# tukaani-project/xz

Measured on AMD Instinct MI355X. Metric: compress MB/s + ratio vs xz -T0 -6, 4 GiB input, 1/2/4/8 MI355X, higher is better.
Workload: dtype u8

## Files before the change

### include/xz_amd.h

```cpp
#ifndef XZ_AMD_H
#define XZ_AMD_H

#include <stddef.h>
#include <stdint.h>

#ifdef __cplusplus
extern "C" {
#endif

typedef struct xzamd_ctx xzamd_ctx;

#define XZAMD_OK              0
#define XZAMD_STREAM_END      1
#define XZAMD_UNSUPPORTED_CHECK 3
#define XZAMD_MEM_ERROR       5
#define XZAMD_OPTIONS_ERROR   8
#define XZAMD_DATA_ERROR      9
#define XZAMD_BUF_ERROR      10
#define XZAMD_PROG_ERROR     11
#define XZAMD_DEVICE_ERROR  100

#define XZAMD_CHECK_NONE   0
#define XZAMD_CHECK_CRC32  1
#define XZAMD_CHECK_CRC64  4
// ... 59 lines not shown
void xzamd_release_parked(void);
uint64_t xzamd_mt_block_size(const xzamd_lzma_options *opt);
uint64_t xzamd_block_buffer_bound(uint64_t uncompressed_size);
uint64_t xzamd_stream_buffer_bound(uint64_t in_size, uint64_t block_size);

int xzamd_ctx_create(xzamd_ctx **ctx, int device);
void xzamd_ctx_destroy(xzamd_ctx *ctx);
int xzamd_ctx_set_batch_bytes(xzamd_ctx *ctx, uint64_t bytes);
const char *xzamd_last_error(const xzamd_ctx *ctx);
int xzamd_ctx_device(const xzamd_ctx *ctx);

typedef struct {
	uint64_t in_bytes, out_bytes;
	uint64_t blocks, spans, batches;
	uint64_t blocks_stored;
	float ms_chains;
	float ms_encode;
	float ms_crc;
	float ms_assemble;
	float ms_total;
	uint32_t encode_launches;
	float ms_find;
	uint32_t span_size;
	float ms_find_overlapped;
	uint32_t span_cost_used;
	float ms_plan;
	uint32_t wave_slots;
	uint64_t enc_spans;
	float ms_seed;
	float ms_parse;
	float ms_code;
	float ms_iter1;
	float ms_verify;
} xzamd_stats;
void xzamd_get_stats(const xzamd_ctx *ctx, xzamd_stats *out);

#define XZAMD_F_BLOCKS_ONLY 1u
#define XZAMD_F_SEGMENTS 2u

#define XZAMD_F_KEEP_RESUME 4u
#define XZAMD_F_VERIFY 8u
#define XZAMD_F_REPAIR 16u
#define XZAMD_F_SINGLE 32u
#define XZAMD_F_AUTO_DELTA 64u

typedef struct {
	uint64_t unpadded_size;
	uint64_t uncompressed_size;
	uint64_t out_offset;
	uint64_t total_size;
} xzamd_block_info;

int xzamd_stream_encode_device(xzamd_ctx *ctx,
		const void *d_in, uint64_t in_size, uint64_t block_size,
		const xzamd_lzma_options *opt, int check, uint32_t flags,
		void *d_out, uint64_t out_cap, uint64_t *out_size,
		xzamd_block_info *binfo, uint64_t binfo_cap, uint64_t *nblocks,
		void *stream);

int xzamd_auto_delta_device(xzamd_ctx *ctx, const void *d_in, uint64_t in_size, uint64_t block_size, uint32_t *dist_out,
		uint64_t cap, uint64_t *nblocks, void *stream);

int xzamd_stream_decode_device(xzamd_ctx *ctx, const void *d_xz, uint64_t xz_size, void *d_out, uint64_t out_cap,
		uint64_t *out_size, const void *d_expected, uint64_t expected_size, uint64_t *mismatches, uint64_t *nblocks,
		void *stream);

// ... 142 lines not shown
```

### xz_amd/__init__.py

```python
import ctypes as C
import os

_HERE = os.path.dirname(os.path.abspath(__file__))
LIB_PATH = os.environ.get("XZ_AMD_LIB") or os.path.join(_HERE, "libxz_amd.so")

CHECK_NONE, CHECK_CRC32, CHECK_CRC64, CHECK_SHA256 = 0, 1, 4, 10
MF_HC3, MF_HC4, MF_BT4 = 0x03, 0x04, 0x14
PRESET_EXTREME = 0x80000000
SPAN_WHOLE_BLOCK = 0xFFFFFFFF
SPAN_DEFAULT = 0
SPAN_AUTO = 1
F_BLOCKS_ONLY = 1
F_SEGMENTS = 2
F_KEEP_RESUME = 4
F_VERIFY = 8
F_REPAIR = 16
F_SINGLE = 32
F_AUTO_DELTA = 64
AUTO_DELTA_DISTANCES = (0, 1, 2, 3, 4, 6, 8, 12, 16, 24, 32)
DEBUG_DELTA_HIST, DEBUG_DELTA_DIST = 19, 20
VSTEPS = ("none", "grammar", "decode", "check", "compare")
NO_BLOCK = 0xFFFFFFFFFFFFFFFF
BCJ_X86 = 4
BCJ_ARM64 = 0x0A
BCJ_RISCV = 0x0B
BCJ_POWERPC, BCJ_IA64, BCJ_ARM, BCJ_ARMTHUMB, BCJ_SPARC = 5, 6, 7, 8, 9


def filter_delta(dist):
    return 3 | ((dist - 1) << 8)



class LzmaOptions(C.Structure):
    _fields_ = [(n, C.c_uint32) for n in (
        "dict_size", "lc", "lp", "pb", "mode", "nice_len", "mf", "depth",
        "gpu_mf", "gpu_nice_len", "gpu_depth", "span_size", "gpu_sa_window", "gpu_parser", "bcj",
        "gpu_sa_depth", "span_cost", "span_bits", "enc_span_bits", "bcj2", "bcj3", "part_iters")]


class Stats(C.Structure):
    _fields_ = [("in_bytes", C.c_uint64), ("out_bytes", C.c_uint64), ("blocks", C.c_uint64),
                ("spans", C.c_uint64), ("batches", C.c_uint64), ("blocks_stored", C.c_uint64),
                ("ms_chains", C.c_float), ("ms_encode", C.c_float), ("ms_crc", C.c_float),
                ("ms_assemble", C.c_float), ("ms_total", C.c_float), ("encode_launches", C.c_uint32),
                ("ms_find", C.c_float), ("span_size", C.c_uint32), ("ms_find_overlapped", C.c_float),
                ("span_cost_used", C.c_uint32), ("ms_plan", C.c_float), ("wave_slots", C.c_uint32),
                ("enc_spans", C.c_uint64), ("ms_seed", C.c_float), ("ms_parse", C.c_float), ("ms_code", C.c_float), ("ms_iter1", C.c_float),
                ("ms_verify", C.c_float)]


class VerifyReport(C.Structure):
    _fields_ = [("units", C.c_uint64), ("blocks", C.c_uint64), ("records_used", C.c_uint64), ("first_bad_block", C.c_uint64),
                ("mismatching_words", C.c_uint64), ("table_used", C.c_uint32), ("first_bad_step", C.c_uint32),
                ("ms_verify", C.c_float), ("reserved_", C.c_uint32)]


class RepairReport(C.Structure):
    _fields_ = [("blocks", C.c_uint64), ("blocks_bad", C.c_uint64), ("blocks_reencoded", C.c_uint64),
                ("blocks_stored", C.c_uint64), ("size_before", C.c_uint64), ("size_after", C.c_uint64),
                ("passes", C.c_uint32), ("ms_repair", C.c_float), ("ms_verify_passes", C.c_float),
                ("ms_reencode", C.c_float), ("ms_splice", C.c_float), ("reserved_", C.c_uint32)]


class ForwardReport(C.Structure):
    _fields_ = [(n, C.c_uint64) for n in ("streams", "blocks", "blocks_delivered", "consumed", "stop_offset")] + \
               [(n, C.c_uint32) for n in ("stop", "code", "step", "reserved_")]


FWD_CONCATENATED = 1
FWD_END, FWD_TRUNCATED, FWD_DEFECT, FWD_OUT_FULL = 1, 2, 3, 4


class BlockInfo(C.Structure):
    _fields_ = [("unpadded_size", C.c_uint64), ("uncompressed_size", C.c_uint64),
                ("out_offset", C.c_uint64), ("total_size", C.c_uint64)]


class XzStream(C.Structure):
    _fields_ = [(n, C.c_uint64) for n in ("offset", "size", "padding", "first_block", "block_count",
                                          "uncompressed_offset", "uncompressed_size")] + \
               [("check", C.c_uint32), ("reserved_", C.c_uint32)]
# ... 527 lines not shown
```

### xz_amd/csrc/xzamd_host.c

```c
#include "../../include/xz_amd.h"
#include "kernels_api.h"
#include "xzamd_internal.h"
#include "delta_rule.h"

#include <stdio.h>
#include <pthread.h>
#include <stdlib.h>
#include <string.h>

#define DEFAULT_BATCH ((1ull << 31) - (1ull << 20))
#define CRC_STRIP 4096u

typedef struct {
	void *p;
	uint64_t cap;
} dbuf;

enum { EV_START, EV_CHAINS, EV_FIND, EV_PLAN0, EV_PLAN1, EV_SEED, EV_ITER1, EV_PARSE, EV_FRONT, EV_BACK0, EV_CODE, EV_CRC, EV_ASM, EV_COUNT };

typedef struct {
	int active;
	uint64_t b0, nb, in_off, n64;
	uint32_t n;
	uint32_t nspans, nenc;
	uint32_t nout, opb;
	uint32_t nch;
	uint64_t sort_bytes;
	int par;
	int sha_early;
	const uint8_t *enc_in;
	uint64_t max_segs, max_lits;
} batch_run;

typedef struct {
	int no_overlap;
	int back_beside_build;
	int timing;
	uint32_t tok_limit, log_cap;
} call_knobs;

typedef struct {
	const xzamd_lzma_options *opt;
	const uint8_t *d_in;
	uint8_t *d_out;
	uint64_t in_size, block_size, out_cap, bound, binfo_cap, total_blocks;
	uint64_t max_blocks;
	uint32_t hb, hmask, hbits;
	uint32_t span;
	uint32_t spb, esb, cpb;
	uint32_t cbytes, hs_fixed;
	uint32_t hs_delta;
	int auto_delta;
	int segments;
	xzamd_mode m;
	call_knobs k;
	int check, whole, filtered, pipelined, defer, seeds_early;
	int resume, verify;
	int repair;
	uint32_t rec_done;
	uint8_t dbyte;
	void *st, *stb;
	uint64_t *rec_unp, *rec_unc;
	xzamd_block_info *binfo;
	uint64_t opos;
} job_env;

struct xzamd_ctx {
	int device;
	void *own_stream;
	void *st2;
	void *st3;
	void *ev_seed[2][3];
	void *ev_sha;
	uint64_t batch_bytes;
	uint32_t wave_slots;
	uint32_t cus;
	uint32_t span_waves;
	uint64_t alloc_limit;
	char err[256];
	char err_msg_buf[200];
	dbuf keys_a, keys_b, vals_a, vals_b, rank, sorted_pos, prev2, prev3, prev4, prev8, prev16, prev24, prev32, key64_a, key64_b, sa, sa_rank, sort_tmp;
	dbuf scratch, span_bytes, strip_crc, block_crc, segs, lits, trace, errw, errw2, litp, mlen, mdist, bcj[2], bcjt;
	dbuf est, totals, span_tab[2], span_cnt[2], mtop, order;
	dbuf pinfo[2], snap_sr, part_tab;
	dbuf cb_bnd[2], cb_log[2], cb_hdr[2], cb_start[2], cb_carry[2];
	dbuf sym_len[2], sym_dist[2], prior, enc_tab[2], enc_cnt[2];
	dbuf tok, chunks, h_chunks;
	dbuf dhist, ddist[2];
	dbuf resume_sr;
	dbuf resume_tab;
	struct { int valid; uint32_t stride, nrec; uint64_t nblocks, block_size, in_size; } resume;
	xzamd_verify_report report;
	xzamd_repair_report repair;
	dbuf h_span_bytes, h_block_crc, h_segs, h_lits, h_span_tab, h_span_cnt[2], h_enc_tab[2], h_enc_cnt[2], h_err[2], h_ddist[2];
	void *evp[2][EV_COUNT];
	void *ev_total[2];
	uint32_t trace_cap;
	int trace_on;
	int last_par;
	struct { int active; job_env J; batch_run B; } pend;
	int pend_has_result, pend_rc;
	uint64_t pend_out_size;
	uint64_t par_seq;
	pthread_mutex_t prog_mu;
// ... 28 lines not shown
		b->p = NULL;
		b->cap = 0;
	}
	bytes = (bytes + 255) & ~255ull;
	if (c->alloc_limit && bytes > c->alloc_limit)
		return fail(c, XZAMD_MEM_ERROR, "allocation above XZAMD_TEST_ALLOC_LIMIT_MIB", 0);
	int e = host ? xzk_host_alloc(&b->p, bytes) : xzk_malloc(&b->p, bytes);
	if (e)
		return fail(c, XZAMD_MEM_ERROR, host ? "hipHostMalloc" : "hipMalloc", e);
	b->cap = bytes;
	return 0;
}

int xzamd_ctx_create(xzamd_ctx **out, int device)
{
	*out = NULL;
	int ndev = 0;
	if (xzk_device_count(&ndev) || ndev <= 0)
		return XZAMD_DEVICE_ERROR;
	xzamd_ctx *c = (xzamd_ctx *)calloc(1, sizeof(*c));
	if (!c)
		return XZAMD_MEM_ERROR;
	if (device < 0) {
		if (xzk_get_device(&device)) { free(c); return XZAMD_DEVICE_ERROR; }
	}
	if (device >= ndev || xzk_set_device(device)) { free(c); return XZAMD_DEVICE_ERROR; }
	c->device = device;
	if (pthread_mutex_init(&c->prog_mu, NULL)) { free(c); return XZAMD_MEM_ERROR; }
	c->prog_mu_ok = 1;
	if (xzk_stream_create(&c->own_stream)) { c->own_stream = NULL; xzamd_ctx_destroy(c); return XZAMD_DEVICE_ERROR; }
	if ((getenv("XZAMD_ST2_LOW") ? xzk_stream_create_low(&c->st2) : xzk_stream_create(&c->st2))) { c->st2 = NULL; xzamd_ctx_destroy(c); return XZAMD_DEVICE_ERROR; }
	if (xzk_event_create(&c->ev_sha)) { c->ev_sha = NULL; xzamd_ctx_destroy(c); return XZAMD_DEVICE_ERROR; }
	if (xzk_stream_create(&c->st3)) { c->st3 = NULL; xzamd_ctx_destroy(c); return XZAMD_DEVICE_ERROR; }
	for (int i = 0; i < 6; ++i)
		if (xzk_event_create(&c->ev_seed[i / 3][i % 3])) { c->ev_seed[i / 3][i % 3] = NULL; xzamd_ctx_destroy(c); return XZAMD_DEVICE_ERROR; }
	for (int i = 0; i < 2 * EV_COUNT; ++i)
		if (xzk_event_create(&c->evp[i / EV_COUNT][i % EV_COUNT])) { c->evp[i / EV_COUNT][i % EV_COUNT] = NULL; xzamd_ctx_destroy(c); return XZAMD_DEVICE_ERROR; }
	for (int i = 0; i < 2; ++i)
		if (xzk_event_create(&c->ev_total[i])) { c->ev_total[i] = NULL; xzamd_ctx_destroy(c); return XZAMD_DEVICE_ERROR; }
	{
		const char *lim = getenv("XZAMD_TEST_ALLOC_LIMIT_MIB");
		c->alloc_limit = (lim && *lim && atoll(lim) > 0) ? (uint64_t)atoll(lim) << 20 : 0;
	}
	c->batch_bytes = DEFAULT_BATCH;
	{
		int cus = 0;
		if (xzk_cu_count(device, &cus) || cus <= 0) cus = 256;
		int occ = 0;
		if (xzk_span_occupancy(1, 64, &occ) || occ <= 0 || occ > 32) occ = 16;
		c->cus = (uint32_t)cus;
		c->wave_slots = (uint32_t)cus * (uint32_t)occ;
		const char *pw = getenv("XZAMD_SPAN_WAVES_PER_CU");
		c->span_waves = (pw && atoi(pw) > 0) ? (uint32_t)cus * (uint32_t)atoi(pw) : 0;
	}
	const char *env = getenv("XZAMD_BATCH_MIB");
	if (env && atoll(env) > 0)
		xzamd_ctx_set_batch_bytes(c, (uint64_t)atoll(env) << 20);
	*out = c;
	return XZAMD_OK;
}

#define CTX_NBUF_MAX 96
static void ctx_device_bufs(xzamd_ctx *c, dbuf **d, size_t *nd)
{
	dbuf *all[] = { &c->keys_a, &c->keys_b, &c->vals_a, &c->vals_b, &c->rank, &c->sorted_pos,
		&c->prev2, &c->prev3, &c->prev4, &c->prev8, &c->prev16, &c->prev24, &c->prev32, &c->key64_a, &c->key64_b, &c->sa, &c->sa_rank, &c->sort_tmp,
// ... 6 lines not shown
		&c->cb_carry[0], &c->cb_carry[1], &c->resume_sr, &c->ddist[0], &c->ddist[1] };
	_Static_assert(sizeof(all) / sizeof(all[0]) <= CTX_NBUF_MAX, "ctx_device_bufs: raise CTX_NBUF_MAX");
	*nd = sizeof(all) / sizeof(all[0]);
	memcpy(d, all, sizeof(all));
}
#define CTX_NBIG 36

void xzamd_ctx_destroy(xzamd_ctx *c)
{
	if (!c)
		return;
	xzk_set_device(c->device);
	if (c->pend.active) {
		if (c->st2) xzk_sync(c->st2);
		c->pend.active = 0;
	}
	dbuf *d[CTX_NBUF_MAX];
	size_t nd = 0;
	ctx_device_bufs(c, d, &nd);
	for (size_t i = 0; i < nd; ++i)
		if (d[i]->p) xzk_free(d[i]->p);
	if (c->resume_tab.p) xzk_free(c->resume_tab.p);
	dbuf *h[] = { &c->h_span_bytes, &c->h_block_crc, &c->h_segs, &c->h_lits, &c->h_span_tab, &c->h_span_cnt[0], &c->h_span_cnt[1],
		&c->h_enc_tab[0], &c->h_enc_tab[1], &c->h_enc_cnt[0], &c->h_enc_cnt[1], &c->h_err[0], &c->h_err[1], &c->h_chunks, &c->h_ddist[0], &c->h_ddist[1] };
	for (size_t i = 0; i < sizeof(h) / sizeof(h[0]); ++i)
		if (h[i]->p) xzk_host_free(h[i]->p);
	for (int i = 0; i < 2 * EV_COUNT; ++i)
		if (c->evp[i / EV_COUNT][i % EV_COUNT]) xzk_event_destroy(c->evp[i / EV_COUNT][i % EV_COUNT]);
	for (int i = 0; i < 2; ++i)
		if (c->ev_total[i]) xzk_event_destroy(c->ev_total[i]);
	if (c->ev_sha) xzk_event_destroy(c->ev_sha);
	for (int i = 0; i < 6; ++i)
		if (c->ev_seed[i / 3][i % 3]) xzk_event_destroy(c->ev_seed[i / 3][i % 3]);
	if (c->st3) xzk_stream_destroy(c->st3);
	if (c->st2) xzk_stream_destroy(c->st2);
	if (c->own_stream) xzk_stream_destroy(c->own_stream);
	if (c->prog_mu_ok) pthread_mutex_destroy(&c->prog_mu);
	free(c);
}

uint64_t xzamd_ctx_progress_in_(xzamd_ctx *c)
{
	if (!c || !c->prog_mu_ok)
		return 0;
	pthread_mutex_lock(&c->prog_mu);
	uint64_t v = c->prog_done;
	if (c->prog_cur) {
		void **ev = c->evp[c->prog_par];
		uint32_t pct = 0;
		if (xzk_event_query(ev[EV_CHAINS]) == 0) {
			pct = 25;
			if (xzk_event_query(ev[EV_FIND]) == 0) {
				pct = 40;
				if (xzk_event_query(ev[EV_PARSE]) == 0)
					pct = xzk_event_query(ev[EV_CODE]) == 0 ? 100 : 90;
			}
		}
		v += c->prog_cur / 100 * pct;
	}
	pthread_mutex_unlock(&c->prog_mu);
	return v;
}

void xzamd_ctx_progress_reset_(xzamd_ctx *c)
{
	if (!c || !c->prog_mu_ok)
// ... 140 lines not shown
	uint8_t *lits; uint64_t lits_len, lits_cap;
	xzamd_copy_seg *segs; uint64_t nsegs, segs_cap;
} plan;

static uint64_t plan_lit(plan *p, const uint8_t *bytes, uint64_t n, uint64_t dst)
{
	memcpy(p->lits + p->lits_len, bytes, n);
	xzamd_copy_seg *s = &p->segs[p->nsegs++];
	s->src = p->lits_len; s->dst = dst; s->len = n; s->kind = 1; s->pad_ = 0;
	p->lits_len += n;
	return dst + n;
}

static uint64_t plan_seg(plan *p, uint32_t kind, uint64_t src, uint64_t n, uint64_t dst)
{
	if (n == 0)
		return dst;
	xzamd_copy_seg *s = &p->segs[p->nsegs++];
	s->src = src; s->dst = dst; s->len = n; s->kind = kind; s->pad_ = 0;
	return dst + n;
}

static uint32_t knob_below(const char *s, uint32_t limit)
{
	const unsigned long v = s ? strtoul(s, NULL, 10) : 0;
	return v >= 1 && v < limit ? (uint32_t)v : 0;
}

static void knobs_read(call_knobs *k)
{
	k->no_overlap = getenv("XZAMD_NO_OVERLAP") != NULL;
	k->back_beside_build = getenv("XZAMD_BACK_BESIDE_BUILD") != NULL;
	k->timing = getenv("XZAMD_TIMING") != NULL;
	k->tok_limit = knob_below(getenv("XZAMD_TEST_TOK_PER_BYTE"), XZAMD_TOK_PER_BYTE);
	k->log_cap = knob_below(getenv("XZAMD_TEST_LOG_CAP"), XZAMD_LOG_CAP);
}

static int call_setup(xzamd_ctx *c, job_env *J, const uint8_t *d_in, uint64_t in_size, uint64_t block_size,
		const xzamd_lzma_options *opt, int check, uint32_t flags, uint8_t *d_out, uint64_t out_cap,
		xzamd_block_info *binfo, uint64_t binfo_cap, void *stream, int may_defer)
{
	if (c->pend_has_result)
		return fail(c, XZAMD_PROG_ERROR, "result of the previous deferred call not collected", 0);
	c->err[0] = 0;
	const uint32_t cbytes = xzamd_check_bytes_(check);
	if (flags & XZAMD_F_SEGMENTS)
		flags |= XZAMD_F_BLOCKS_ONLY;
	if ((unsigned)check > 15)
		return fail(c, XZAMD_PROG_ERROR, "check id out of range", 0);
	const int chains = (flags & XZAMD_F_CHAINS_) != 0;
	if (flags & XZAMD_F_AUTO_DELTA) {
		if (!xzk_delta_stats || !xzk_delta_choose || !xzk_delta_blocks)
			return fail(c, XZAMD_OPTIONS_ERROR, "auto delta: this build has no kernels for it", 0);
		if (opt->bcj != 0)
			return fail(c, XZAMD_OPTIONS_ERROR, "auto delta: the chain already has a filter in front of LZMA2", 0);
		if (flags & XZAMD_F_SEGMENTS)
			return fail(c, XZAMD_OPTIONS_ERROR, "auto delta: Blocks only -- the segments of one Block share its chain", 0);
		if (flags & XZAMD_F_REPAIR)
			return fail(c, XZAMD_OPTIONS_ERROR, "auto delta: not with XZAMD_F_REPAIR (the repair plans Block Headers from one chain)", 0);
	}
	if (chains && (!(flags & XZAMD_F_SEGMENTS) || !xzamd_chains_encoded_))
		return fail(c, XZAMD_OPTIONS_ERROR, "chains: this build has no unit for bare chunk chains", 0);
	if ((flags & XZAMD_F_REPAIR) && (flags & XZAMD_F_SEGMENTS) && !chains)
		return fail(c, XZAMD_OPTIONS_ERROR, "repair: Blocks only, not the chunk chains of XZAMD_F_SEGMENTS", 0);
	if ((flags & (XZAMD_F_KEEP_RESUME | XZAMD_F_VERIFY)) && (flags & XZAMD_F_BLOCKS_ONLY) && !(flags & XZAMD_F_REPAIR) && !chains)
		return fail(c, XZAMD_OPTIONS_ERROR, "keep_resume / verify need a whole Stream: not with XZAMD_F_BLOCKS_ONLY or XZAMD_F_SEGMENTS", 0);
// ... 49 lines not shown
	{
		double per_byte = xzamd_work_bytes_per_byte_(opt);
		if (flags & XZAMD_F_AUTO_DELTA) per_byte += xzamd_auto_delta_bytes_per_byte_(block_size);
		if ((flags & (XZAMD_F_KEEP_RESUME | XZAMD_F_VERIFY)) && J->m.two)
			per_byte += (double)(XZAMD_RESUME_BYTES(J->m.model_slots) + 32u) * (double)(block_size / XZAMD_ENC_MIN_LEN + 1) / (double)block_size;
		uint64_t free_b = 0, total_b = 0, held = 0;
		if (xzk_mem_info(&free_b, &total_b) == 0 && total_b != 0) {
			dbuf *d[CTX_NBUF_MAX];
			size_t nd = 0;
			ctx_device_bufs(c, d, &nd);
			for (size_t i = 0; i < nd; ++i) held += d[i]->cap;
			const double budget = 0.80 * (double)(free_b + held);
			uint64_t fit = (uint64_t)(budget / per_byte) / block_size;
			if (fit == 0) fit = 1;
			if (fit < max_blocks) max_blocks = fit;
		}
	}
	if (total_blocks > max_blocks) {
		const uint64_t nbatch = (total_blocks + max_blocks - 1) / max_blocks;
		max_blocks = (total_blocks + nbatch - 1) / nbatch;
	}
	const int adaptive = J->m.adaptive, two = J->m.two;
	J->spb = adaptive ? (uint32_t)(block_size / XZAMD_SPAN_MIN_LEN + 2) : (uint32_t)((block_size + J->span - 1) / J->span);
	J->esb = two ? (uint32_t)(block_size / XZAMD_ENC_MIN_LEN + 1) : 0;
	J->cpb = (uint32_t)((block_size + XZAMD_EST_CHUNK - 1) / XZAMD_EST_CHUNK);
	J->filtered = opt->bcj != 0;
	J->auto_delta = (flags & XZAMD_F_AUTO_DELTA) != 0;
	const int overlap_ok = two && !J->k.no_overlap;
	J->defer = may_defer && overlap_ok && (flags & XZAMD_F_BLOCKS_ONLY) && total_blocks > 0 && !(flags & (XZAMD_F_REPAIR | XZAMD_F_VERIFY));
	if (c->pend.active && !(overlap_ok && c->pend.J.st == st))
		(void)pend_complete(c);
	J->pipelined = overlap_ok && (total_blocks > max_blocks || J->defer || c->pend.active);
	J->seeds_early = overlap_ok && block_size >= XZAMD_SEED_LEN + 1024;

	J->opt = opt; J->d_in = d_in; J->d_out = d_out; J->in_size = in_size; J->block_size = block_size; J->out_cap = out_cap;
	J->total_blocks = total_blocks; J->max_blocks = max_blocks;
	J->bound = xzamd_block_buffer_bound(block_size);
	J->binfo = binfo; J->binfo_cap = binfo_cap;
	J->cbytes = cbytes; J->hs_fixed = xzamd_block_header_size_(J->bound, block_size, opt);
	if (J->auto_delta) {
		xzamd_lzma_options view = *opt;
		view.bcj = XZAMD_FILTER_DELTA(1);
		J->hs_delta = xzamd_block_header_size_(J->bound, block_size, &view);
	}
	J->check = check;
	J->dbyte = xzamd_dict_size_byte_(opt->dict_size);
	J->st = st; J->stb = J->pipelined ? c->st2 : st;
	J->whole = !(flags & XZAMD_F_BLOCKS_ONLY);
	J->segments = (flags & XZAMD_F_SEGMENTS) != 0;
	J->resume = (flags & (XZAMD_F_KEEP_RESUME | XZAMD_F_VERIFY)) && two;
	J->verify = (flags & XZAMD_F_VERIFY) != 0;
	J->repair = (flags & XZAMD_F_REPAIR) != 0;
	c->resume.valid = 0;
	if (c->resume_tab.p && !J->resume && !c->pend.active) {
		xzk_free(c->resume_tab.p);
		c->resume_tab.p = NULL; c->resume_tab.cap = 0;
	}
	if (J->resume) {
		const uint64_t cap = total_blocks * J->esb;
		if (cap >= 0xFFFFFFFFull)
			return fail(c, XZAMD_OPTIONS_ERROR, "too many encode spans for a resume table", 0);
		int r = dgrow(c, &c->resume_tab, (cap ? cap : 1) * XZAMD_RESUME_BYTES(J->m.model_slots), 0);
		if (r) return r;
	}

	memset(&c->stats, 0, sizeof(c->stats));
// ... 45 lines not shown
	B->nb = J->total_blocks - b0 < J->max_blocks ? J->total_blocks - b0 : J->max_blocks;
	B->in_off = b0 * block_size;
	const uint64_t n64 = J->in_size - B->in_off < B->nb * block_size ? J->in_size - B->in_off : B->nb * block_size;
	B->n = (uint32_t)n64;
	B->n64 = B->n;
	uint32_t bb = 0;
	while ((1u << bb) < B->nb + 1) ++bb;
	const uint32_t bits[4] = { 10 + bb, 16 + bb, J->hbits + bb, 32 };
	for (int i = 0; i < 4; ++i) {
		uint64_t sbytes = 0;
		int e = xzk_sort_temp_bytes(B->n, bits[i], &sbytes);
		if (e)
			return fail(c, XZAMD_DEVICE_ERROR, "rocprim temp size", e);
		if (sbytes > B->sort_bytes) B->sort_bytes = sbytes;
	}
	if (J->opt->gpu_sa_window) {
		uint64_t sbytes = 0;
		int e = xzk_sa_temp_bytes(B->n, &sbytes);
		if (e)
			return fail(c, XZAMD_DEVICE_ERROR, "rocprim temp size (suffix order)", e);
		if (sbytes > B->sort_bytes) B->sort_bytes = sbytes;
	}
	B->nspans = (uint32_t)(B->nb * J->spb);
	B->nenc = (uint32_t)(B->nb * J->esb);
	B->nout = J->m.two ? B->nenc : B->nspans;
	B->opb = J->m.two ? J->esb : J->spb;
	B->nch = J->m.two ? XZAMD_CHUNK_SLOTS(B->n, B->nenc) : 0;
	const uint64_t segs_per_block = (J->m.two ? (block_size >> 13) + 2ull * J->esb + 2 : B->opb) + 2 + 2 * ((block_size + 65535) / 65536) + 2;
	B->max_segs = B->nb * segs_per_block + 4;
	B->max_lits = B->nb * (64 + 3 * ((block_size + 65535) / 65536) + 32) + 64;
	return XZAMD_OK;
}

static int batch_reserve(xzamd_ctx *c, const job_env *J, const batch_run *B)
{
	const xzamd_lzma_options *opt = J->opt;
	const int two = J->m.two, par = B->par;
	const uint64_t n = B->n, nb = B->nb, nspans = B->nspans, nenc = B->nenc, nout = B->nout, nch = B->nch;
	const uint64_t mslots = J->m.model_slots;
	const uint64_t spb_crc = (J->block_size + CRC_STRIP - 1) / CRC_STRIP;
	int r = 0;
#define NEED(buf, bytes, host) (r = r ? r : dgrow(c, &c->buf, (bytes), host))
	NEED(keys_a, 4 * n, 0); NEED(keys_b, 4 * n, 0);
	NEED(vals_a, 4 * n, 0); NEED(vals_b, 4 * n, 0);
	NEED(prev2, 4 * n, 0); NEED(prev3, 4 * n, 0);
	if (opt->gpu_sa_window) {
		NEED(prev4, 4 * n, 0); NEED(prev8, 8 * n, 0); NEED(prev16, 8 * n, 0);
		NEED(prev24, 4 * n, 0); NEED(prev32, 4 * n, 0);
		NEED(key64_a, 8 * n, 0); NEED(key64_b, 8 * n, 0);
		NEED(sa, 4 * n, 0); NEED(sa_rank, 4 * n, 0);
	} else {
		NEED(rank, 4 * n, 0); NEED(sorted_pos, 4 * n, 0);
	}
	NEED(sort_tmp, B->sort_bytes + 256, 0);
	NEED(scratch, two ? n + (n >> 3) + 64 + 32 * nch : n + (n >> 3) + 32 + XZAMD_SPAN_SLACK * nout, 0);
	NEED(span_bytes, 4 * nout, 0);
	NEED(span_tab[par], 8 * nspans, 0);
	NEED(span_cnt[par], 4 * nb, 0);
	NEED(h_span_tab, 8 * nspans, 1);
	NEED(h_span_cnt[par], 4 * nb + 16, 1);
	if (two) {
		NEED(sym_len[par], 2 * n + 64, 0);
		NEED(sym_dist[par], 4 * n + 64, 0);
		NEED(prior, 4ull * XZAMD_PRIOR_WORDS * nspans, 0);
		NEED(enc_tab[par], 8 * nenc, 0);
		NEED(enc_cnt[par], 4 * nb, 0);
		NEED(h_enc_tab[par], 8 * nenc, 1);
		NEED(h_enc_cnt[par], 4 * nb + 16, 1);
		NEED(tok, 2 * (n * XZAMD_TOK_PER_BYTE + 4096 * nenc + 64), 0);
		NEED(pinfo[par], 4ull * XZAMD_PINFO_WORDS * nspans, 0);
		NEED(snap_sr, 32 * nspans, 0);
		NEED(part_tab, 4 * nspans + 16, 0);
		for (int f = 0; f < 2; ++f) {
			NEED(cb_bnd[f], 4 * mslots * nenc, 0);
			NEED(cb_log[f], 4ull * XZAMD_LOG_WORDS * mslots * nenc, 0);
// ... 334 lines not shown
	return XZAMD_OK;
}

static void back_stats(xzamd_ctx *c, const job_env *J, const batch_run *B)
{
	const int par = B->par;
	const uint64_t nb = B->nb;
	const uint32_t *hcnt = (const uint32_t *)c->h_span_cnt[par].p;
	float ms;
	void **ev = c->evp[par];
	if (!xzk_event_elapsed_ms(ev[EV_START], ev[EV_CHAINS], &ms)) c->stats.ms_chains += ms;
	if (!xzk_event_elapsed_ms(ev[EV_CHAINS], ev[EV_FRONT], &ms)) c->stats.ms_encode += ms;
	if (J->opt->gpu_parser && !xzk_event_elapsed_ms(ev[EV_CHAINS], ev[EV_FIND], &ms)) c->stats.ms_find += ms;
	if (!xzk_event_elapsed_ms(ev[EV_PLAN0], ev[EV_PLAN1], &ms)) c->stats.ms_plan += ms;
	if (!xzk_event_elapsed_ms(ev[EV_CODE], ev[EV_CRC], &ms)) c->stats.ms_crc += ms;
	if (!xzk_event_elapsed_ms(ev[EV_CRC], ev[EV_ASM], &ms)) c->stats.ms_assemble += ms;
	c->stats.blocks += nb;
	for (uint64_t b = 0; b < nb; ++b) c->stats.spans += hcnt[b];
	if (J->m.two) {
		const uint32_t *ecnt = (const uint32_t *)c->h_enc_cnt[par].p;
		for (uint64_t b = 0; b < nb; ++b) c->stats.enc_spans += ecnt[b];
		if (J->seeds_early) { if (!xzk_event_elapsed_ms(c->ev_seed[par][1], c->ev_seed[par][2], &ms)) c->stats.ms_seed += ms; }
		else if (!xzk_event_elapsed_ms(ev[EV_PLAN1], ev[EV_SEED], &ms)) c->stats.ms_seed += ms;
		if (!xzk_event_elapsed_ms(ev[EV_SEED], ev[EV_PARSE], &ms)) c->stats.ms_parse += ms;
		if (!xzk_event_elapsed_ms(ev[EV_SEED], ev[EV_ITER1], &ms)) c->stats.ms_iter1 += ms;
		if (!xzk_event_elapsed_ms(ev[EV_BACK0], ev[EV_CODE], &ms)) { c->stats.ms_code += ms; c->stats.ms_encode += ms; }
	}
	if (J->m.adaptive) {
		uint64_t tgt;
		memcpy(&tgt, hcnt + 2 * ((nb + 1) / 2), 8);
		c->stats.span_cost_used = tgt > 0xFFFFFFFFull ? 0xFFFFFFFFu : (uint32_t)tgt;
	}
	c->stats.batches += 1;
	c->stats.encode_launches += 1;
}

static int back_finish(xzamd_ctx *c, job_env *J, batch_run *B)
{
	B->active = 0;
	int rc = back_report(c, J, B);
	if (rc != XZAMD_OK) return rc;

	plan pl;
	pl.lits = (uint8_t *)c->h_lits.p; pl.lits_len = 0; pl.lits_cap = B->max_lits;
	pl.segs = (xzamd_copy_seg *)c->h_segs.p; pl.nsegs = 0; pl.segs_cap = B->max_segs;
	uint64_t opos = J->opos;
	for (uint64_t b = 0; b < B->nb; ++b) {
		int stored = 0;
		rc = layout_block(c, J, B, &pl, b, &opos, &stored);
		if (rc != XZAMD_OK) return rc;
		if (J->resume) {
			const uint32_t cnt = ((const uint32_t *)c->h_enc_cnt[B->par].p)[b];
			if (stored)
				for (uint32_t k = 0; k < cnt; ++k)
					if (xzk_memset((uint8_t *)c->resume_tab.p + (uint64_t)(J->rec_done + k) * XZAMD_RESUME_BYTES(J->m.model_slots)
							+ XZAMD_RESUME_KIND_OFF, (int)XZAMD_RK_VOID, 1, J->stb))
						return fail(c, XZAMD_DEVICE_ERROR, "memset resume record", 1);
			J->rec_done += cnt;
		}
	}
	J->opos = opos;
	if (pl.nsegs > pl.segs_cap || pl.lits_len > pl.lits_cap) return fail(c, XZAMD_PROG_ERROR, "plan overflow", 0);

	int e = xzk_h2d(c->segs.p, pl.segs, pl.nsegs * sizeof(xzamd_copy_seg), J->stb);
	if (!e) e = xzk_h2d(c->lits.p, pl.lits, pl.lits_len ? pl.lits_len : 1, J->stb);
	if (!e) e = xzk_assemble((const xzamd_copy_seg *)c->segs.p, (uint32_t)pl.nsegs,
// ... 12 lines not shown
	if (rc == XZAMD_OK) progress_set(c, c->prog_done + n64, 0, 0);
	return rc;
}

static int pend_complete(xzamd_ctx *c)
{
	if (!c->pend.active)
		return XZAMD_OK;
	c->pend.active = 0;
	int rc = back_finish(c, &c->pend.J, &c->pend.B);
	if (rc != XZAMD_OK) xzk_sync(c->st2);
	c->pend_rc = rc;
	c->pend_out_size = c->pend.J.opos;
	c->pend_has_result = 1;
	return rc;
}

int xzamd_encode_finish_(xzamd_ctx *c, uint64_t *out_size)
{
	if (!c || !out_size)
		return XZAMD_PROG_ERROR;
	if (!c->pend_has_result && c->pend.active) {
		xzk_set_device(c->device);
		pend_complete(c);
	}
	if (!c->pend_has_result)
		return fail(c, XZAMD_PROG_ERROR, "no deferred call to finish", 0);
	c->pend_has_result = 0;
	*out_size = c->pend_out_size;
	return c->pend_rc;
}


static int front_input(xzamd_ctx *c, const job_env *J, batch_run *B)
{
	const uint8_t *in = J->d_in + B->in_off;
	const uint32_t n = B->n, bs = (uint32_t)J->block_size, nb = (uint32_t)B->nb;
	void *st = J->st;
	B->enc_in = in;
	xzk_event_record(c->evp[B->par][EV_START], st);
	if (J->check == XZAMD_CHECK_SHA256 && !J->pipelined) {
		int e3 = xzk_stream_wait_event(c->st2, c->evp[B->par][EV_START]);
		if (!e3) e3 = xzk_sha256_blocks(in, n, bs, nb, (uint8_t *)c->block_crc.p, c->st2);
		if (!e3) e3 = xzk_event_record(c->ev_sha, c->st2);
		if (e3) return fail(c, XZAMD_DEVICE_ERROR, "sha256 launch", e3);
		B->sha_early = 1;
	}
	if (J->filtered) {
		uint32_t pre[XZAMD_PREFILTERS_MAX];
		const uint32_t npre = xzamd_prefilter_list_(J->opt, pre);
		uint8_t *const X = (uint8_t *)c->bcj[B->par].p, *const T = (uint8_t *)c->bcjt.p;
		const uint8_t *src = in;
		for (uint32_t i = 0; i < npre; ++i) {
			uint8_t *dst = ((npre - 1 - i) & 1) ? T : X;
			int e = pre[i] == XZAMD_BCJ_X86
					? xzk_x86_bcj(src, dst, n, bs, nb, st)
					: xzk_prefilter(src, dst, n, bs, nb, pre[i] & 0xFF, (pre[i] >> 8) + 1, st);
			if (e) return fail(c, XZAMD_DEVICE_ERROR, "filter in front of LZMA2", e);
			src = dst;
		}
		B->enc_in = X;
	}
	if (J->auto_delta) {
		uint8_t *const X = (uint8_t *)c->bcj[B->par].p;
		uint32_t *const dist = (uint32_t *)c->ddist[B->par].p;
		int e = xzk_delta_stats(in, n, bs, nb, (uint32_t *)c->dhist.p, st);
		if (!e) e = xzk_delta_choose((const uint32_t *)c->dhist.p, nb, dist, st);
		if (!e) e = xzk_delta_blocks(in, X, n, bs, nb, dist, st);
		if (!e) e = xzk_d2h(c->h_ddist[B->par].p, dist, 4ull * nb, st);
		if (e) return fail(c, XZAMD_DEVICE_ERROR, "automatic delta filter", e);
		B->enc_in = X;
	}
	return XZAMD_OK;
}

static int front_build(xzamd_ctx *c, const job_env *J, const batch_run *B, back_args *prev_back)
{
	const xzamd_lzma_options *opt = J->opt;
	void **ev = c->evp[B->par];
#define SA(buf) (opt->gpu_sa_window ? c->buf.p : NULL)
	int e = xzk_build_chains(B->enc_in, B->n, (uint32_t)J->block_size, (uint32_t)B->nb, J->hb, J->hmask, J->hbits, opt->gpu_sa_depth,
			(uint32_t *)c->keys_a.p, (uint32_t *)c->keys_b.p, (uint32_t *)c->vals_a.p,
			(uint32_t *)c->vals_b.p, c->sort_tmp.p, B->sort_bytes,
			(uint32_t *)c->rank.p, (uint32_t *)c->sorted_pos.p, (uint32_t *)c->prev2.p, (uint32_t *)c->prev3.p,
			(uint32_t *)SA(prev4), (uint64_t *)SA(prev8), (uint64_t *)SA(prev16), (uint64_t *)SA(key64_a), (uint64_t *)SA(key64_b),
			(uint32_t *)SA(sa), (uint32_t *)SA(sa_rank), (uint32_t *)SA(prev24), (uint32_t *)SA(prev32), J->st);
#undef SA
	if (e) return fail(c, XZAMD_DEVICE_ERROR, "build_chains", e);
	xzk_event_record(ev[EV_CHAINS], J->st);
	if (!prev_back->valid)
		return XZAMD_OK;
	e = J->stb != J->st ? xzk_stream_wait_event(J->stb, ev[EV_CHAINS]) : 0;
	if (e) return fail(c, XZAMD_DEVICE_ERROR, "stream wait", e);
	return back_enqueue(c, J, prev_back);
}

static int find_part(xzamd_ctx *c, const job_env *J, const xzamd_span_args *a, int part)
{
	return xzk_find_matches(a, (const uint32_t *)c->sa.p, (const uint32_t *)c->sa_rank.p, (const uint32_t *)c->prev4.p,
			(const uint64_t *)c->prev8.p, (const uint64_t *)c->prev16.p,
			(const uint32_t *)c->prev24.p, (const uint32_t *)c->prev32.p, (uint16_t *)a->mlen, (uint32_t *)a->mdist, part, J->st);
}

static int front_find(xzamd_ctx *c, const job_env *J, const batch_run *B, const xzamd_span_args *a)
{
	const int par = B->par;
	if (xzk_memset(c->errw.p, 0, 512, J->st)) return fail(c, XZAMD_DEVICE_ERROR, "memset", 1);
	if (J->opt->gpu_parser) {
		int e = 0;
		if (J->seeds_early) {
			e = find_part(c, J, a, 1);
			if (!e) e = xzk_event_record(c->ev_seed[par][0], J->st);
			if (!e) e = xzk_stream_wait_event(c->st3, c->ev_seed[par][0]);
			if (!e) e = xzk_event_record(c->ev_seed[par][1], c->st3);
			if (!e) e = xzk_parse_pieces(a, (uint32_t)B->nb, 0, 0, NULL, c->st3);
			if (!e) e = xzk_event_record(c->ev_seed[par][2], c->st3);
		}
		if (!e) e = find_part(c, J, a, J->seeds_early ? 2 : 0);
		if (e) return fail(c, XZAMD_DEVICE_ERROR, "find_matches launch", e);
	}
	xzk_event_record(c->evp[par][EV_FIND], J->st);
	return XZAMD_OK;
}

static int front_plan(xzamd_ctx *c, const job_env *J, const batch_run *B, xzamd_span_args *a)
{
	const xzamd_lzma_options *opt = J->opt;
// ... 29 lines not shown
			const uint64_t bs = b * block_size, be = B->n64 - bs < block_size ? B->n64 : bs + block_size;
			uint32_t k = 0;
			for (uint64_t p = bs; p < be; p += span, ++k) {
				htab[2 * (b * spb + k)] = (uint32_t)p;
				htab[2 * (b * spb + k) + 1] = (uint32_t)(be - p < span ? be : p + span);
			}
			hcnt[b] = k;
		}
		e = xzk_h2d(c->span_tab[par].p, htab, 8ull * B->nspans, st);
		if (!e) e = xzk_h2d(c->span_cnt[par].p, hcnt, 4ull * nb, st);
		if (e) return fail(c, XZAMD_DEVICE_ERROR, "h2d span plan", e);
	}
	xzk_event_record(ev[EV_PLAN1], st);
	return XZAMD_OK;
}

static int front_parse(xzamd_ctx *c, const job_env *J, const batch_run *B, xzamd_span_args *a)
{
	const int par = B->par;
	const uint32_t nb = (uint32_t)B->nb;
	void *st = J->st;
	void **ev = c->evp[par];
	uint32_t *const counter = (uint32_t *)c->errw.p + 60;
	int e;
	if (J->m.two) {
		if (J->seeds_early) e = xzk_stream_wait_event(st, c->ev_seed[par][2]);
		else e = xzk_parse_pieces(a, nb, 0, 0, NULL, st);
		xzk_event_record(ev[EV_SEED], st);
		const uint32_t npart = J->opt->part_iters ? J->opt->part_iters : XZAMD_PART_ITERS_DEFAULT;
		for (uint32_t it = 0; it < npart && !e; ++it) {
			a->iter = XZAMD_ITER_PARTIAL | (it ? XZAMD_ITER_SNAP : 0u);
			if (it) e = xzk_memset(counter, 0, 4, st);
			if (!e) e = xzk_parse_pieces(a, nb, 1, c->span_waves, counter, st);
			if (!e) e = xzk_model_snapshots(a, nb, st);
		}
		xzk_event_record(ev[EV_ITER1], st);
		a->iter = XZAMD_ITER_SNAP;
		if (!e) e = xzk_memset(counter, 0, 4, st);
		if (!e) e = xzk_parse_pieces(a, nb, 1, c->span_waves, counter, st);
		xzk_event_record(ev[EV_PARSE], st);
	} else {
		e = xzk_span_encode(a, B->nspans, c->span_waves, counter, st);
		xzk_event_record(ev[EV_PARSE], st);
	}
	if (e) return fail(c, XZAMD_DEVICE_ERROR, "span_encode launch", e);
	e = xzk_d2h(c->h_err[par].p, c->errw.p, 512, st);
	if (e) return fail(c, XZAMD_DEVICE_ERROR, "d2h", e);
	xzk_event_record(ev[EV_FRONT], st);
	return XZAMD_OK;
}


static int back_stage(xzamd_ctx *c, job_env *J, batch_run *cur, const xzamd_span_args *a, back_args *BA, batch_run *prev)
{
	int rc;
	if (J->pipelined && c->pend.active) {
		(void)pend_complete(c);
	} else if (J->pipelined && prev->active) {
		rc = back_finish_own(c, J, prev);
		if (rc != XZAMD_OK) return rc;
	}
	BA->valid = 1;
	BA->a = *a;
	BA->B = *cur;
	if (!(!J->k.back_beside_build && J->pipelined && cur->b0 + cur->nb < J->total_blocks)) {
		rc = back_enqueue(c, J, BA);
		if (rc != XZAMD_OK) return rc;
	}
	progress_set(c, c->prog_done, cur->n64, cur->par);
	if (J->pipelined) {
		*prev = *cur;
		return XZAMD_OK;
	}
	return back_finish_own(c, J, cur);
}

static int batches_drain_release(xzamd_ctx *c, job_env *J, back_args *BA, batch_run *prev)
{
	int rc;
	c->err[0] = 0;
	if (c->pend.active)
		(void)pend_complete(c);
	if (BA->valid) {
		rc = back_enqueue(c, J, BA);
		if (rc != XZAMD_OK) return rc;
	}
	if (prev->active) {
		rc = back_finish_own(c, J, prev);
		if (rc != XZAMD_OK) return rc;
	}
	xzk_sync(J->st);
	xzk_sync(c->st2);
	dbuf *d[CTX_NBUF_MAX];
	size_t nd = 0;
	ctx_device_bufs(c, d, &nd);
	for (size_t i = 0; i < CTX_NBIG && i < nd; ++i)
		if (d[i]->p) { xzk_free(d[i]->p); d[i]->p = NULL; d[i]->cap = 0; }
	return XZAMD_OK;
}

int xzamd_stream_encode_device(xzamd_ctx *c,
		const void *d_in_, uint64_t in_size, uint64_t block_size,
		const xzamd_lzma_options *opt, int check, uint32_t flags,
		void *d_out_, uint64_t out_cap, uint64_t *out_size,
		xzamd_block_info *binfo, uint64_t binfo_cap, uint64_t *nblocks_out,
		void *stream)
{
	if (c && (flags & XZAMD_F_CHAINS_))
		return fail(c, XZAMD_OPTIONS_ERROR, "unknown flag", 0);
	if (c && (flags & XZAMD_F_SINGLE) && (flags & XZAMD_F_AUTO_DELTA))
		return fail(c, XZAMD_OPTIONS_ERROR, "auto delta: Blocks only -- the single Block of XZAMD_F_SINGLE has one chain", 0);
	if (c && (flags & XZAMD_F_SINGLE)) {
		if (!xzamd_single_encode_)
			return fail(c, XZAMD_OPTIONS_ERROR, "single: this build has no unit for bare chunk chains", 0);
		return xzamd_single_encode_(c, d_in_, in_size, block_size, opt, check, flags & ~XZAMD_F_SINGLE, d_out_, out_cap, out_size, binfo,
				binfo_cap, nblocks_out, stream);
	}
	return xzamd_encode_device_(c, d_in_, in_size, block_size, opt, check, flags, d_out_, out_cap, out_size, binfo, binfo_cap,
			nblocks_out, stream, NULL);
}

int xzamd_auto_delta_device(xzamd_ctx *c, const void *d_in_, uint64_t in_size, uint64_t block_size, uint32_t *dist_out, uint64_t cap,
		uint64_t *nblocks_out, void *stream)
{
	if (!c || (!d_in_ && in_size) || !nblocks_out || (!dist_out && cap))
// ... 28 lines not shown
		if (!e) e = xzk_sync(st);
		if (e) return fail(c, XZAMD_DEVICE_ERROR, "automatic delta analysis", e);
	}
	return XZAMD_OK;
}

int xzamd_encode_device_(xzamd_ctx *c,
		const void *d_in_, uint64_t in_size, uint64_t block_size,
		const xzamd_lzma_options *opt, int check, uint32_t flags,
		void *d_out_, uint64_t out_cap, uint64_t *out_size,
		xzamd_block_info *binfo, uint64_t binfo_cap, uint64_t *nblocks_out,
		void *stream, int *deferred)
{
	if (deferred) *deferred = 0;
	if (!c || !opt || !out_size || (!d_in_ && in_size) || !d_out_)
		return XZAMD_PROG_ERROR;
	job_env J;
	memset(&J, 0, sizeof(J));
	int rc = call_setup(c, &J, (const uint8_t *)d_in_, in_size, block_size, opt, check, flags, (uint8_t *)d_out_, out_cap,
			binfo, binfo_cap, stream, deferred != NULL);
	if (rc != XZAMD_OK)
		return rc;
	if (nblocks_out) *nblocks_out = J.total_blocks;
	if (J.whole) {
		rc = stream_begin(c, &J);
		if (rc != XZAMD_OK)
			return rc;
	}

	batch_run prev;
	memset(&prev, 0, sizeof(prev));
	back_args BA;
	memset(&BA, 0, sizeof(BA));
	progress_set(c, 0, 0, 0);
	xzk_event_record(c->ev_total[0], J.st);
	for (uint64_t b0 = 0; b0 < J.total_blocks && rc == XZAMD_OK; ) {
		batch_run cur;
		xzamd_span_args a;
		rc = batch_geometry(c, &J, b0, &cur);
		if (rc != XZAMD_OK) break;
		cur.par = J.pipelined ? (int)(c->par_seq++ & 1) : 0;
		rc = batch_reserve(c, &J, &cur);
		if (rc == XZAMD_MEM_ERROR && cur.nb > 1) {
			J.max_blocks = (cur.nb + 1) / 2;
			rc = batches_drain_release(c, &J, &BA, &prev);
			continue;
		}
		if (rc != XZAMD_OK) break;
		cur.active = 1;
		c->last_par = cur.par;

		rc = front_input(c, &J, &cur);
		if (rc == XZAMD_OK) rc = front_build(c, &J, &cur, &BA);
		if (rc == XZAMD_OK) {
			span_args_init(c, &J, &cur, &a);
			rc = front_find(c, &J, &cur, &a);
		}
		if (rc == XZAMD_OK) rc = front_plan(c, &J, &cur, &a);
		if (rc == XZAMD_OK) rc = front_parse(c, &J, &cur, &a);
		if (rc == XZAMD_OK) rc = back_stage(c, &J, &cur, &a, &BA, &prev);
		b0 += cur.nb;
	}
	if (rc == XZAMD_OK && c->pend.active)
		(void)pend_complete(c);
	if (rc == XZAMD_OK && prev.active) {
		if (J.defer) {
			c->pend.J = J;
			c->pend.B = prev;
			c->pend.active = 1;
			prev.active = 0;
			*deferred = 1;
		} else {
			rc = back_finish_own(c, &J, &prev);
		}
	}
	if (rc != XZAMD_OK && c->pend.active)
		pend_complete(c);
	xzk_sync(J.st);
	xzk_sync(c->st3);
	if (!(deferred && *deferred))
		xzk_sync(c->st2);
	if (rc == XZAMD_OK && J.whole)
		rc = stream_end(c, &J);
	xzk_event_record(c->ev_total[1], J.st);
	xzk_sync(J.st);
	{
		float ms;
		if (!xzk_event_elapsed_ms(c->ev_total[0], c->ev_total[1], &ms)) c->stats.ms_total = ms;
	}
	free(J.rec_unp);
	c->stats.in_bytes = in_size;
	c->stats.out_bytes = J.opos;
	*out_size = (deferred && *deferred) ? 0 : J.opos;
	if (rc == XZAMD_OK && J.resume) {
		c->resume.valid = 1;
		c->resume.stride = XZAMD_RESUME_BYTES(J.m.model_slots); c->resume.nrec = J.rec_done;
		c->resume.nblocks = J.total_blocks; c->resume.block_size = J.block_size; c->resume.in_size = in_size;
	}
	if (rc == XZAMD_OK && J.segments && J.verify) {
		uint64_t ns = J.opos;
		rc = xzamd_chains_encoded_(c, J.d_out, J.opos, J.out_cap, J.d_in, in_size, J.opt, J.check, J.repair, J.binfo, J.total_blocks,
				&ns, J.st);
		if (rc == XZAMD_OK) {
			*out_size = ns;
			c->stats.out_bytes = ns;
		}
		c->stats.ms_verify = c->report.ms_verify;
	} else if (rc == XZAMD_OK && J.repair) {
		uint64_t ns = J.opos;
		rc = xzamd_repair_encoded_(c, J.d_out, J.opos, J.out_cap, J.d_in, in_size, J.block_size, J.opt, J.check, J.whole, J.binfo,
				J.binfo_cap, J.total_blocks, &ns, J.st);
		if (rc == XZAMD_OK) {
// ... 11 lines not shown
```

Baseline: 653.9.

## Build next batch's match chains ahead on a side stream during parse

```diff
diff --git a/include/xz_amd.h b/include/xz_amd.h
--- a/include/xz_amd.h
+++ b/include/xz_amd.h
@@ -115,6 +115,7 @@
 	float ms_code;
 	float ms_iter1;
 	float ms_verify;
+	uint32_t batches_ahead;
 } xzamd_stats;
 void xzamd_get_stats(const xzamd_ctx *ctx, xzamd_stats *out);
 
diff --git a/xz_amd/__init__.py b/xz_amd/__init__.py
--- a/xz_amd/__init__.py
+++ b/xz_amd/__init__.py
@@ -47,7 +47,7 @@
                 ("ms_find", C.c_float), ("span_size", C.c_uint32), ("ms_find_overlapped", C.c_float),
                 ("span_cost_used", C.c_uint32), ("ms_plan", C.c_float), ("wave_slots", C.c_uint32),
                 ("enc_spans", C.c_uint64), ("ms_seed", C.c_float), ("ms_parse", C.c_float), ("ms_code", C.c_float), ("ms_iter1", C.c_float),
-                ("ms_verify", C.c_float)]
+                ("ms_verify", C.c_float), ("batches_ahead", C.c_uint32)]
 
 
 class VerifyReport(C.Structure):
diff --git a/xz_amd/csrc/xzamd_host.c b/xz_amd/csrc/xzamd_host.c
--- a/xz_amd/csrc/xzamd_host.c
+++ b/xz_amd/csrc/xzamd_host.c
@@ -16,7 +16,7 @@
 	uint64_t cap;
 } dbuf;
 
-enum { EV_START, EV_CHAINS, EV_FIND, EV_PLAN0, EV_PLAN1, EV_SEED, EV_ITER1, EV_PARSE, EV_FRONT, EV_BACK0, EV_CODE, EV_CRC, EV_ASM, EV_COUNT };
+enum { EV_START, EV_CHAINS, EV_FIND, EV_PLAN0, EV_PLAN1, EV_SEED, EV_PART, EV_ITER1, EV_PARSE, EV_FRONT, EV_BACK0, EV_CODE, EV_CRC, EV_ASM, EV_COUNT };
 
 typedef struct {
 	int active;
@@ -28,13 +28,18 @@
 	uint64_t sort_bytes;
 	int par;
 	int sha_early;
+	int ahead;
 	const uint8_t *enc_in;
 	uint64_t max_segs, max_lits;
 } batch_run;
 
+enum { AHEAD_PLAN = 1, AHEAD_PART, AHEAD_ITER1 };
+#define AHEAD_DEFAULT AHEAD_PLAN
+
 typedef struct {
 	int no_overlap;
 	int back_beside_build;
+	int build_ahead;
 	int timing;
 	uint32_t tok_limit, log_cap;
 } call_knobs;
@@ -55,11 +60,13 @@
 	xzamd_mode m;
 	call_knobs k;
 	int check, whole, filtered, pipelined, defer, seeds_early;
+	int ahead;
 	int resume, verify;
 	int repair;
 	uint32_t rec_done;
 	uint8_t dbyte;
 	void *st, *stb;
+	void *sta;
 	uint64_t *rec_unp, *rec_unc;
 	xzamd_block_info *binfo;
 	uint64_t opos;
@@ -70,6 +77,7 @@
 	void *own_stream;
 	void *st2;
 	void *st3;
+	void *st4;
 	void *ev_seed[2][3];
 	void *ev_sha;
 	uint64_t batch_bytes;
@@ -164,6 +172,13 @@
 	if ((getenv("XZAMD_ST2_LOW") ? xzk_stream_create_low(&c->st2) : xzk_stream_create(&c->st2))) { c->st2 = NULL; xzamd_ctx_destroy(c); return XZAMD_DEVICE_ERROR; }
 	if (xzk_event_create(&c->ev_sha)) { c->ev_sha = NULL; xzamd_ctx_destroy(c); return XZAMD_DEVICE_ERROR; }
 	if (xzk_stream_create(&c->st3)) { c->st3 = NULL; xzamd_ctx_destroy(c); return XZAMD_DEVICE_ERROR; }
+	{
+		const char *sv = getenv("XZAMD_BUILD_AHEAD_STREAM");
+		const int low = sv && !strcmp(sv, "low");
+		if ((low || (sv && !strcmp(sv, "own"))) && (low ? xzk_stream_create_low(&c->st4) : xzk_stream_create(&c->st4))) {
+			c->st4 = NULL; xzamd_ctx_destroy(c); return XZAMD_DEVICE_ERROR;
+		}
+	}
 	for (int i = 0; i < 6; ++i)
 		if (xzk_event_create(&c->ev_seed[i / 3][i % 3])) { c->ev_seed[i / 3][i % 3] = NULL; xzamd_ctx_destroy(c); return XZAMD_DEVICE_ERROR; }
 	for (int i = 0; i < 2 * EV_COUNT; ++i)
@@ -236,6 +251,7 @@
 	if (c->ev_sha) xzk_event_destroy(c->ev_sha);
 	for (int i = 0; i < 6; ++i)
 		if (c->ev_seed[i / 3][i % 3]) xzk_event_destroy(c->ev_seed[i / 3][i % 3]);
+	if (c->st4) xzk_stream_destroy(c->st4);
 	if (c->st3) xzk_stream_destroy(c->st3);
 	if (c->st2) xzk_stream_destroy(c->st2);
 	if (c->own_stream) xzk_stream_destroy(c->own_stream);
@@ -442,6 +458,11 @@
 	k->no_overlap = getenv("XZAMD_NO_OVERLAP") != NULL;
 	k->back_beside_build = getenv("XZAMD_BACK_BESIDE_BUILD") != NULL;
 	k->timing = getenv("XZAMD_TIMING") != NULL;
+	{
+		const char *ba = getenv("XZAMD_BUILD_AHEAD");
+		k->build_ahead = !ba || !*ba ? AHEAD_DEFAULT : !strcmp(ba, "plan") ? AHEAD_PLAN : !strcmp(ba, "part") ? AHEAD_PART
+				: !strcmp(ba, "iter1") ? AHEAD_ITER1 : !strcmp(ba, "0") ? 0 : AHEAD_DEFAULT;
+	}
 	k->tok_limit = knob_below(getenv("XZAMD_TEST_TOK_PER_BYTE"), XZAMD_TOK_PER_BYTE);
 	k->log_cap = knob_below(getenv("XZAMD_TEST_LOG_CAP"), XZAMD_LOG_CAP);
 }
@@ -557,6 +578,8 @@
 		(void)pend_complete(c);
 	J->pipelined = overlap_ok && (total_blocks > max_blocks || J->defer || c->pend.active);
 	J->seeds_early = overlap_ok && block_size >= XZAMD_SEED_LEN + 1024;
+	J->ahead = J->pipelined && opt->gpu_parser ? J->k.build_ahead : 0;
+	J->sta = c->st4 ? c->st4 : c->st3;
 
 	J->opt = opt; J->d_in = d_in; J->d_out = d_out; J->in_size = in_size; J->block_size = block_size; J->out_cap = out_cap;
 	J->total_blocks = total_blocks; J->max_blocks = max_blocks;
@@ -668,7 +691,7 @@
 	return XZAMD_OK;
 }
 
-static int batch_reserve(xzamd_ctx *c, const job_env *J, const batch_run *B)
+static int batch_reserve(xzamd_ctx *c, const job_env *J, const batch_run *B, int probe)
 {
 	const xzamd_lzma_options *opt = J->opt;
 	const int two = J->m.two, par = B->par;
@@ -676,7 +699,7 @@
 	const uint64_t mslots = J->m.model_slots;
 	const uint64_t spb_crc = (J->block_size + CRC_STRIP - 1) / CRC_STRIP;
 	int r = 0;
-#define NEED(buf, bytes, host) (r = r ? r : dgrow(c, &c->buf, (bytes), host))
+#define NEED(buf, bytes, host) (r = r ? r : probe ? c->buf.cap < (uint64_t)(bytes) : dgrow(c, &c->buf, (bytes), host))
 	NEED(keys_a, 4 * n, 0); NEED(keys_b, 4 * n, 0);
 	NEED(vals_a, 4 * n, 0); NEED(vals_b, 4 * n, 0);
 	NEED(prev2, 4 * n, 0); NEED(prev3, 4 * n, 0);
@@ -1077,6 +1100,7 @@
 		c->stats.span_cost_used = tgt > 0xFFFFFFFFull ? 0xFFFFFFFFu : (uint32_t)tgt;
 	}
 	c->stats.batches += 1;
+	c->stats.batches_ahead += B->ahead != 0;
 	c->stats.encode_launches += 1;
 }
 
@@ -1155,11 +1179,10 @@
 }
 
 
-static int front_input(xzamd_ctx *c, const job_env *J, batch_run *B)
+static int front_input(xzamd_ctx *c, const job_env *J, batch_run *B, void *st)
 {
 	const uint8_t *in = J->d_in + B->in_off;
 	const uint32_t n = B->n, bs = (uint32_t)J->block_size, nb = (uint32_t)B->nb;
-	void *st = J->st;
 	B->enc_in = in;
 	xzk_event_record(c->evp[B->par][EV_START], st);
 	if (J->check == XZAMD_CHECK_SHA256 && !J->pipelined) {
@@ -1197,25 +1220,61 @@
 	return XZAMD_OK;
 }
 
-static int front_build(xzamd_ctx *c, const job_env *J, const batch_run *B, back_args *prev_back)
+static int build_launch(xzamd_ctx *c, const job_env *J, const batch_run *B, void *st)
 {
 	const xzamd_lzma_options *opt = J->opt;
-	void **ev = c->evp[B->par];
 #define SA(buf) (opt->gpu_sa_window ? c->buf.p : NULL)
 	int e = xzk_build_chains(B->enc_in, B->n, (uint32_t)J->block_size, (uint32_t)B->nb, J->hb, J->hmask, J->hbits, opt->gpu_sa_depth,
 			(uint32_t *)c->keys_a.p, (uint32_t *)c->keys_b.p, (uint32_t *)c->vals_a.p,
 			(uint32_t *)c->vals_b.p, c->sort_tmp.p, B->sort_bytes,
 			(uint32_t *)c->rank.p, (uint32_t *)c->sorted_pos.p, (uint32_t *)c->prev2.p, (uint32_t *)c->prev3.p,
 			(uint32_t *)SA(prev4), (uint64_t *)SA(prev8), (uint64_t *)SA(prev16), (uint64_t *)SA(key64_a), (uint64_t *)SA(key64_b),
-			(uint32_t *)SA(sa), (uint32_t *)SA(sa_rank), (uint32_t *)SA(prev24), (uint32_t *)SA(prev32), J->st);
+			(uint32_t *)SA(sa), (uint32_t *)SA(sa_rank), (uint32_t *)SA(prev24), (uint32_t *)SA(prev32), st);
 #undef SA
 	if (e) return fail(c, XZAMD_DEVICE_ERROR, "build_chains", e);
-	xzk_event_record(ev[EV_CHAINS], J->st);
+	xzk_event_record(c->evp[B->par][EV_CHAINS], st);
+	return XZAMD_OK;
+}
+
+static int front_build(xzamd_ctx *c, const job_env *J, const batch_run *B, back_args *prev_back)
+{
+	void **ev = c->evp[B->par];
+	int e = 0;
+	if (B->ahead) {
+		e = xzk_stream_wait_event(J->st, ev[EV_CHAINS]);
+		if (e) return fail(c, XZAMD_DEVICE_ERROR, "stream wait", e);
+	} else {
+		int rc = build_launch(c, J, B, J->st);
+		if (rc != XZAMD_OK) return rc;
+	}
 	if (!prev_back->valid)
 		return XZAMD_OK;
 	e = J->stb != J->st ? xzk_stream_wait_event(J->stb, ev[EV_CHAINS]) : 0;
 	if (e) return fail(c, XZAMD_DEVICE_ERROR, "stream wait", e);
 	return back_enqueue(c, J, prev_back);
+}
+
+static int ahead_issue(xzamd_ctx *c, const job_env *J, const batch_run *cur, batch_run *next)
+{
+	memset(next, 0, sizeof(*next));
+	const uint64_t b0 = cur->b0 + cur->nb;
+	if (!J->ahead || b0 >= J->total_blocks)
+		return XZAMD_OK;
+	batch_run N;
+	int rc = batch_geometry(c, J, b0, &N);
+	if (rc != XZAMD_OK) return rc;
+	N.par = (int)(c->par_seq & 1);
+	if (batch_reserve(c, J, &N, 1))
+		return XZAMD_OK;
+	void **evc = c->evp[cur->par];
+	int e = xzk_stream_wait_event(J->sta, evc[J->ahead == AHEAD_PLAN ? EV_PLAN1 : J->ahead == AHEAD_PART ? EV_PART : EV_ITER1]);
+	if (e) return fail(c, XZAMD_DEVICE_ERROR, "stream wait", e);
+	++c->par_seq;
+	N.ahead = 1;
+	*next = N;
+	rc = front_input(c, J, next, J->sta);
+	if (rc == XZAMD_OK) rc = build_launch(c, J, next, J->sta);
+	return rc;
 }
 
 static int find_part(xzamd_ctx *c, const job_env *J, const xzamd_span_args *a, int part)
@@ -1311,6 +1370,7 @@
 			a->iter = XZAMD_ITER_PARTIAL | (it ? XZAMD_ITER_SNAP : 0u);
 			if (it) e = xzk_memset(counter, 0, 4, st);
 			if (!e) e = xzk_parse_pieces(a, nb, 1, c->span_waves, counter, st);
+			if (J->ahead == AHEAD_PART && it + 1 == npart) xzk_event_record(ev[EV_PART], st);
 			if (!e) e = xzk_model_snapshots(a, nb, st);
 		}
 		xzk_event_record(ev[EV_ITER1], st);
@@ -1370,6 +1430,7 @@
 	}
 	xzk_sync(J->st);
 	xzk_sync(c->st2);
+	xzk_sync(J->sta);
 	dbuf *d[CTX_NBUF_MAX];
 	size_t nd = 0;
 	ctx_device_bufs(c, d, &nd);
@@ -1464,25 +1525,32 @@
 	memset(&prev, 0, sizeof(prev));
 	back_args BA;
 	memset(&BA, 0, sizeof(BA));
+	batch_run next;
+	memset(&next, 0, sizeof(next));
 	progress_set(c, 0, 0, 0);
 	xzk_event_record(c->ev_total[0], J.st);
 	for (uint64_t b0 = 0; b0 < J.total_blocks && rc == XZAMD_OK; ) {
 		batch_run cur;
 		xzamd_span_args a;
-		rc = batch_geometry(c, &J, b0, &cur);
-		if (rc != XZAMD_OK) break;
-		cur.par = J.pipelined ? (int)(c->par_seq++ & 1) : 0;
-		rc = batch_reserve(c, &J, &cur);
-		if (rc == XZAMD_MEM_ERROR && cur.nb > 1) {
-			J.max_blocks = (cur.nb + 1) / 2;
-			rc = batches_drain_release(c, &J, &BA, &prev);
-			continue;
-		}
-		if (rc != XZAMD_OK) break;
+		if (next.ahead) {
+			cur = next;
+			next.ahead = 0;
+		} else {
+			rc = batch_geometry(c, &J, b0, &cur);
+			if (rc != XZAMD_OK) break;
+			cur.par = J.pipelined ? (int)(c->par_seq++ & 1) : 0;
+			rc = batch_reserve(c, &J, &cur, 0);
+			if (rc == XZAMD_MEM_ERROR && cur.nb > 1) {
+				J.max_blocks = (cur.nb + 1) / 2;
+				rc = batches_drain_release(c, &J, &BA, &prev);
+				continue;
+			}
+			if (rc != XZAMD_OK) break;
+		}
 		cur.active = 1;
 		c->last_par = cur.par;
 
-		rc = front_input(c, &J, &cur);
+		if (!cur.ahead) rc = front_input(c, &J, &cur, J.st);
 		if (rc == XZAMD_OK) rc = front_build(c, &J, &cur, &BA);
 		if (rc == XZAMD_OK) {
 			span_args_init(c, &J, &cur, &a);
@@ -1491,6 +1559,7 @@
 		if (rc == XZAMD_OK) rc = front_plan(c, &J, &cur, &a);
 		if (rc == XZAMD_OK) rc = front_parse(c, &J, &cur, &a);
 		if (rc == XZAMD_OK) rc = back_stage(c, &J, &cur, &a, &BA, &prev);
+		if (rc == XZAMD_OK) rc = ahead_issue(c, &J, &cur, &next);
 		b0 += cur.nb;
 	}
 	if (rc == XZAMD_OK && c->pend.active)
@@ -1510,6 +1579,7 @@
 		pend_complete(c);
 	xzk_sync(J.st);
 	xzk_sync(c->st3);
+	if (J.sta != c->st3) xzk_sync(J.sta);
 	if (!(deferred && *deferred))
 		xzk_sync(c->st2);
 	if (rc == XZAMD_OK && J.whole)
```

Result: faster. 681.6 (median of 6 runs) (+4.2%).
